# WISDEM/RAFT

Hardware: AMD Instinct MI355X
Metric: design-case-frequency solves/sec (whole node) (higher is better)
Workload: dtype f64

## Files before the change

raft_amd/_abi.py:

```python
import ctypes as C
import os

import numpy as np

NFIELD = 32
FLAG_CONVERGED = 1
FLAG_NAN = 2

_c_double_p = C.POINTER(C.c_double)
_c_i64_p = C.POINTER(C.c_int64)
_c_i32_p = C.POINTER(C.c_int32)
_vp = C.c_void_p

EXPORTS = (
    "raftx_version", "raftx_is_device", "raftx_ctx_create", "raftx_ctx_destroy",
    "raftx_last_error", "raftx_upload_designs", "raftx_upload_cases",
    "raftx_excitation", "raftx_linearize", "raftx_solve_dynamics",
    "raftx_solve_system", "raftx_last_kernel_ms",
    "raftx_solve_dynamics_device", "raftx_fetch_results", "raftx_debug_math", "raftx_debug_math_table", "raftx_last_solve_kernel", "raftx_device_synchronize", "raftx_motion_stats", "raftx_solve_system_resident", "raftx_qtf_slender", "raftx_channel_stats", "raftx_qtf_force", "raftx_set_linearisation_point", "raftx_fetch_linearisation_point",
    "raftx_build_designs", "raftx_fetch_strips", "raftx_fetch_statics", "raftx_channel_stats_poly", "raftx_qtf_slender_rows", "raftx_bem_excitation", "raftx_qtf_kay", "raftx_host_alloc", "raftx_host_free", "raftx_device_locality", "raftx_solve_dense",
    "raftx_sweep_stats",
    "raftx_sweep_submit",
    "raftx_sweep_prepare",
    "raftx_sweep_launch",
# ... 115 lines not shown
            L.raftx_modal_batch.argtypes = [_vp, C.c_int, _vp, _vp, _vp, _vp, _vp]
            L.raftx_modal_batch.restype = C.c_int
            L.raftx_modal_resident.argtypes = [_vp, _vp, _vp, _vp, _vp, _vp, _vp]
            L.raftx_modal_resident.restype = C.c_int
            L.raftx_sweep_modal.argtypes = [_vp, C.c_int, _vp, _vp, _vp, _vp, _vp, _vp]
            L.raftx_sweep_modal.restype = C.c_int
        self.has_mooring = all(hasattr(L, s) for s in MOORING_EXPORTS)
        if self.has_mooring:
            L.raftx_mooring_lines.argtypes = [_vp, C.c_int, C.c_int, _vp, _vp, C.c_double, _vp, _vp, _vp, _vp, _vp, _vp]
            L.raftx_mooring_lines.restype = C.c_int
            L.raftx_mooring_program.argtypes = [_vp, C.c_int, _vp, C.c_int, _vp, _vp]
            L.raftx_mooring_program.restype = C.c_int
            L.raftx_mooring_expand.argtypes = [_vp, C.c_int, _vp, _vp]
            L.raftx_mooring_expand.restype = C.c_int
            L.raftx_sweep_mooring.argtypes = [_vp, C.c_int, C.c_int, _vp, C.c_int, _vp, _vp, _vp, _vp, _vp]
            L.raftx_sweep_mooring.restype = C.c_int
        self.has_statics = all(hasattr(L, s) for s in STATICS_EXPORTS)
        if self.has_statics:
            L.raftx_mean_pose.argtypes = [_vp, C.c_int, C.c_int, _vp, _vp, C.c_double, _vp, _vp, _vp, _vp, _vp, C.c_int,
                                          _vp, _vp, _vp, _vp, _vp, _vp, _vp, _vp]
            L.raftx_mean_pose.restype = C.c_int
            L.raftx_sweep_mean_pose.argtypes = [_vp, C.c_int, C.c_int, _vp, C.c_int, _vp, _vp, _vp, _vp, C.c_int, _vp, _vp, _vp, _vp]
            L.raftx_sweep_mean_pose.restype = C.c_int
        self.has_current = all(hasattr(L, s) for s in CURRENT_EXPORTS)
        if self.has_current:
            L.raftx_current_loads.argtypes = [_vp, C.c_int, _vp, _vp, _vp, C.c_double, C.c_double, _vp]
            L.raftx_current_loads.restype = C.c_int
            L.raftx_sweep_current.argtypes = [_vp, C.c_int, C.c_int, _vp, _vp, _vp, C.c_double, _vp]
            L.raftx_sweep_current.restype = C.c_int
        self.has_qtfgen = all(hasattr(L, s) for s in QTFGEN_EXPORTS)
        if self.has_qtfgen:
            L.raftx_qtf_tables_build.argtypes = [_vp, C.c_int, _vp, _vp, _vp, _vp, _vp, _vp, _vp]
            L.raftx_qtf_tables_build.restype = C.c_int
            L.raftx_qtf_tables_build_variants.argtypes = [_vp, C.c_int, _vp, _vp, _vp, _vp]
            L.raftx_qtf_tables_build_variants.restype = C.c_int
            L.raftx_qtf_tables_counts.argtypes = [_vp, _vp]
            L.raftx_qtf_tables_counts.restype = C.c_int
            L.raftx_qtf_tables_fetch.argtypes = [_vp, _vp, _vp, _vp, _vp]
            L.raftx_qtf_tables_fetch.restype = C.c_int
            L.raftx_qtf_tables_kay_items.argtypes = [_vp, C.c_int, _vp, _vp, _vp]
            L.raftx_qtf_tables_kay_items.restype = C.c_int
            L.raftx_qtf_slender_resident.argtypes = [_vp, C.c_int, C.c_int, _vp, _vp, C.c_double, C.c_double, C.c_double, _vp, _vp,
                                                     _vp, C.c_int, _vp]
            L.raftx_qtf_slender_resident.restype = C.c_int
        self.has_channels = all(hasattr(L, s) for s in CHANNEL_EXPORTS)
        if self.has_channels:
# ... 345 lines not shown
                                                        float(XiStart), int(n_chunk), _ptr(out["std"]), _ptr(out["niter"]),
                                                        _ptr(out["flags"]), _ptr(out["Xi"]), _ptr(out["strip_off"]))
        self._check(rc, "raftx_sweep_prepare_variants")
        return dict(slot=int(slot), inputs=inputs, out=out)

    def sweep_launch(self, handle):
        self._check(self.rlib.lib.raftx_sweep_launch(self._h, int(handle["slot"])), "raftx_sweep_launch")
        return handle

    def sweep_submit(self, slot, *args, **kw):
        return self.sweep_launch(self.sweep_prepare(slot, *args, **kw))

    def sweep_wait(self, handle):
        out = handle["out"]
        self._check(self.rlib.lib.raftx_sweep_wait(self._h, int(handle["slot"]), _ptr(out["timing_ms"])), "raftx_sweep_wait")
        span = np.zeros(2)
        self._check(self.rlib.lib.raftx_sweep_solve_span(self._h, int(handle["slot"]), _ptr(span[0:1]), _ptr(span[1:2])),
                    "raftx_sweep_solve_span")
        out["solve_span_ms"] = span
        nf, nb = C.c_int(0), C.c_int(0)
        self._check(self.rlib.lib.raftx_sweep_generation(self._h, int(handle["slot"]), C.byref(nf), C.byref(nb)),
                    "raftx_sweep_generation")
        out["generation_fused_blocks"] = (nf.value, nb.value)
        handle["inputs"] = None
        return out

    def sweep_cancel(self, handle):
        self._check(self.rlib.lib.raftx_sweep_cancel(self._h, int(handle["slot"])), "raftx_sweep_cancel")
        handle["inputs"] = None

    def sweep_stats(self, tables, M0, B0, C0, w, k, depth, zeta, beta, nIter, tol=0.01, XiStart=0.1, pose=None,
                    rho=1025.0, g=9.81, rho_wave=1025.0, g_wave=9.81, add_mask=7, Fz_moor=None, n_chunk=0, n_worker=0,
                    want_Xi=False, Xi_out=None):
        self.resident_generation += 1
        nD, nC, nH, nw, inputs, out = self._sweep_prepare(tables, M0, B0, C0, w, k, depth, zeta, beta, pose, Fz_moor, want_Xi, Xi_out)
        (member_off, members, station_off, stations, cap_off, caps, pose, M0, B0, C0, Fz, w, k, zeta, beta) = inputs
        rc = self.rlib.lib.raftx_sweep_stats(self._h, nD, _ptr(member_off), _ptr(members), _ptr(station_off), _ptr(stations),
                                             _ptr(cap_off), _ptr(caps), _ptr(pose), float(rho), float(g), int(add_mask),
                                             _ptr(M0), _ptr(B0), _ptr(C0), _ptr(Fz), nC, nH, nw, _ptr(w), _ptr(k), float(depth),
                                             float(rho_wave), float(g_wave), _ptr(zeta), _ptr(beta), int(nIter), float(tol),
                                             float(XiStart), int(n_chunk), int(n_worker), _ptr(out["std"]), _ptr(out["niter"]),
                                             _ptr(out["flags"]), _ptr(out["Xi"]), _ptr(out["strip_off"]), _ptr(out["timing_ms"]))
        self._check(rc, "raftx_sweep_stats")
        return out

    def fetch_strips(self, n_strips, n_cm_rows=0):
# ... 819 lines not shown
```

raft_amd/csrc/build.py:

```python
import os
import subprocess
import sys

HERE = os.path.dirname(os.path.abspath(__file__))
SRC = os.path.join(HERE, "raftx_hip.hip")
OUT = os.path.join(HERE, "libraftx_hip.so")
FLAGS = ["--offload-arch=gfx950", "-O3", "-std=c++17", "-shared", "-fPIC", "-fno-gpu-rdc", "-mllvm", "-disable-machine-licm"]


def build(force=False, verbose=False, extra=()):
    deps = [SRC, os.path.join(HERE, "..", "..", "include", "raftx.h"), os.path.join(HERE, "..", "..", "include", "raftx_modal.h"),
            os.path.join(HERE, "..", "..", "include", "raftx_current.h"),
            os.path.join(HERE, "..", "..", "include", "raftx_channels.h"),
            os.path.join(HERE, "..", "..", "include", "raftx_qtfgen.h"),
            os.path.join(HERE, "..", "..", "include", "raftx_mooring.h"),
            os.path.join(HERE, "..", "..", "include", "raftx_statics.h"), os.path.abspath(__file__)]
    deps += [os.path.join(HERE, f) for f in os.listdir(HERE) if f.endswith(".h")]
    if (not force) and os.path.exists(OUT) and all(os.path.getmtime(OUT) >= os.path.getmtime(d) for d in deps):
        return OUT
    hipcc = os.environ.get("HIPCC", "hipcc")
    cmd = [hipcc] + FLAGS + list(extra) + ["-o", OUT, SRC]
    if verbose:
        print(" ".join(cmd))
    subprocess.check_call(cmd)
    return OUT


def build_timing(verbose=False):
    out = os.path.join(HERE, "libraftx_hip_timing.so")
    cmd = [os.environ.get("HIPCC", "hipcc")] + FLAGS + ["-DRAFTX_PHASE_TIMING", "-DGEOM_PHASE_TIMING", "-o", out, SRC]
    if verbose:
        print(" ".join(cmd))
    subprocess.check_call(cmd)
    return out


if __name__ == "__main__":
    if "--timing" in sys.argv:
        print(build_timing(verbose=True))
# ... 4 lines not shown
```

raft_amd/csrc/raftx_hip.hip:

```cpp

#include <hip/hip_runtime.h>
#include <rccl/rccl.h>
#include <dlfcn.h>

#include <algorithm>
#include <cmath>
#include <cstdint>
#include <cstdio>
#include <cstdlib>
#include <cstring>
#include <chrono>
#include <map>
#include <functional>
#include <limits>
#include <mutex>
#include <type_traits>
#include <thread>
#include <unordered_map>
#include <vector>

#include "../../include/raftx.h"
#include "../../include/raftx_modal.h"
#include "../../include/raftx_current.h"
#include "../../include/raftx_channels.h"
#include "../../include/raftx_qtfgen.h"
#include "../../include/raftx_mooring.h"
#include "../../include/raftx_statics.h"

struct Roctx {
    int (*push)(const char *) = nullptr;
    int (*pop)() = nullptr;
    Roctx() {
        if (getenv("RAFTX_NO_ROCTX")) return;
        for (const char *n : {"librocprofiler-sdk-roctx.so.1", "librocprofiler-sdk-roctx.so", "libroctx64.so.4", "libroctx64.so"}) {
            if (void *h = dlopen(n, RTLD_NOW | RTLD_LOCAL)) {
                push = reinterpret_cast<int (*)(const char *)>(dlsym(h, "roctxRangePushA"));
                pop = reinterpret_cast<int (*)()>(dlsym(h, "roctxRangePop"));
                if (push && pop) return;
                push = nullptr;
                pop = nullptr;
            }
        }
    }
};
static Roctx &roctx() {
    static Roctx r;
    return r;
}
struct RangeScope {
    bool on;
// ... 296 lines not shown
    const size_t t = (size_t)blockIdx.x * blockDim.x + threadIdx.x;
    if (t >= (size_t)npair * 36 * nw) return;
    const int iw = (int)(t % nw), e = (int)((t / nw) % 36);
    const size_t pair = t / ((size_t)36 * nw), d = pair / nCase;
    const double ww = w[iw], Bq = uB[d * 36 + e] + uBd[pair * 36 + e];
    Z[t] = {fma(-(ww * ww), uM[d * 36 + e], uC[d * 36 + e]), ww * Bq};
}

static int solve_system_shape(int n, int nRhs, size_t *lds) {
    const size_t per = sizeof(cplx) * (size_t)n * (n + nRhs);
    const int nbin = per * 4 <= 64 * 1024 ? 4 : (per * 2 <= 64 * 1024 ? 2 : 1);
    *lds = per * nbin;
    return nbin;
}

__global__ void __launch_bounds__(256) k_motion_stats(int npair, int nHead, int nw, double inv_dw,
                                                      const cplx *__restrict__ Xi, double *__restrict__ sd,
                                                      double *__restrict__ psd,
                                                      const int *__restrict__ niter = nullptr, const int *__restrict__ flags = nullptr,
                                                      int *__restrict__ ints_out = nullptr) {
    __shared__ double part[4][6];
    const int p = blockIdx.x;
    if (p >= npair) return;
    const double r2d = 180.0 / 3.14159265358979323846;
    double acc[6] = {0, 0, 0, 0, 0, 0};
    for (int i = threadIdx.x; i < nw; i += blockDim.x) {
#pragma unroll
        for (int j = 0; j < 6; j++) {
            const double scale = j >= 3 ? r2d : 1.0;
            double a2 = 0.0;
            for (int ih = 0; ih < nHead; ih++) {
                const cplx x = Xi[(((size_t)p * nHead + ih) * 6 + j) * nw + i];
                const double xr = x.re * scale, xi = x.im * scale;
                a2 += xr * xr + xi * xi;
            }
            acc[j] += a2;
            if (psd) psd[((size_t)p * 6 + j) * nw + i] = 0.5 * a2 * inv_dw;
        }
    }
    const int lane = threadIdx.x & 63, wv = threadIdx.x >> 6;
#pragma unroll
    for (int j = 0; j < 6; j++) {
        double a = acc[j];
        for (int o = 32; o > 0; o >>= 1) a += __shfl_xor(a, o, 64);
        if (lane == 0) part[wv][j] = a;
    }
    __syncthreads();
    if (threadIdx.x < 6) {
        double a = 0.0;
        for (int q = 0; q < (int)(blockDim.x >> 6); q++) a += part[q][threadIdx.x];
        sd[(size_t)p * 6 + threadIdx.x] = sqrt(0.5 * a);
    }
    if (ints_out && threadIdx.x == 6) {
        ints_out[p] = niter[p];
        ints_out[npair + p] = flags[p];
    }
}

// ... 242 lines not shown
};
struct VariantSrc {
    const VariantProg *prog;
    const double *params;
    const FixedRecord *rec = nullptr;
};

static void variant_view(const VariantProg &P, VariantView &V) {
    V.nM = P.nM; V.nSt = P.nSt; V.nCap = P.nCap; V.nP = P.nP;
    V.gm = P.gm; V.gs = P.gs; V.gc = P.gc;
    V.stMember = P.stMember; V.capMember = P.capMember;
    V.stFrac = P.stFrac; V.fillFrac = P.fillFrac; V.capFrac = P.capFrac;
    V.endCoef = P.endCoef; V.headCS = P.headCS; V.diaCoef = P.diaCoef;
    V.endEdit = P.endEdit; V.diaEdit = P.diaEdit;
}
static void expand_args(const VariantProg &P, int n, double *gm_out, double *gs_out, double *gc_out, ExpandArgs &E) {
    variant_view(P, E);
    E.n = n;
    E.gm_out = gm_out; E.gs_out = gs_out; E.gc_out = gc_out;
}
static bool fused_gen_asked() {
    const char *fg = getenv("RAFTX_FUSED_GEN");
    return fg && atoi(fg);
}

struct DenseResident {
    int nSet = 0, n = 0, nw = 0, freq_mask = 0;
    double *w = nullptr, *M = nullptr, *B = nullptr, *C = nullptr;
    Bag allocs;
};
struct QtfResident {
    bool valid = false;
    int nDesign = 0;
    std::vector<int64_t> off;
    int64_t *dOff = nullptr;
    double *strips = nullptr, *members = nullptr, *kay = nullptr;
    Bag allocs;
    int64_t total(int j) const { return off[(size_t)j * (nDesign + 1) + nDesign]; }
};
struct raftx_ctx;
struct DevOffsets {
    const int64_t *memberOff, *stationOff, *capOff;
};
struct SeaStates { int nCase, nHead, nw; const double *w, *k; double depth, rho, g; const double *zeta, *beta; };
struct BuildSource {
    const int64_t *memberOff, *stationOff, *capOff;
// ... 163 lines not shown
    DevTables T{};
    cplx *rXi = nullptr, *rFw = nullptr, *rZ = nullptr, *rFe = nullptr;
    double *rB = nullptr;
    int *rNi = nullptr, *rFl = nullptr;
    size_t r_npair = 0, r_nx = 0, r_nz = 0;
    int r_mask = 0;
    int r_last_mask = 0;
    bool r_fe = false;
    unsigned kpNext = 0;
    int nCU = 0;
    int last_flags = -1, last_minb = 0, last_rc = 0;
    int rQtf_sets = 0, rQtf_nw2 = 0, rKay_sets = 0, rKay_nw2 = 0;
    bool have_xl0 = false, want_xlout = false;
    int maxS = 0;
    std::vector<int> hS;
    double last_ms = 0.0;
    bool have_designs = false, have_cases = false;
    int nw_designs = 0;
    bool kay_ready = false, bem_ready = false;
    int g_n = 0;
    size_t g_nStrips = 0, g_nRows = 0;
    double *g_abi = nullptr, *g_A = nullptr, *g_Ch = nullptr, *g_Wh = nullptr, *g_props = nullptr, *g_Ms = nullptr, *g_Cs = nullptr, *g_Ws = nullptr;
    bool last_gen_fused = false;
    cplx *g_cm = nullptr;
    void *comm = nullptr;
    int comm_rank = 0, comm_world = 1;
    std::vector<raftx_ctx *> workers[RAFTX_NSLOT];
};

#define MAX_NW 2048
#define HIPCHK(ctx, call)                                                                              \
    do {                                                                                               \
        hipError_t e_ = (call);                                                                        \
        if (e_ != hipSuccess) {                                                                        \
            snprintf((ctx)->err, sizeof((ctx)->err), "%s failed: %s (%s:%d)", #call, hipGetErrorString(e_), \
                     __FILE__, __LINE__);                                                              \
            return -2;                                                                                 \
        }                                                                                              \
    } while (0)
#define FAIL(ctx, ...)                                        \
    do {                                                      \
        snprintf((ctx)->err, sizeof((ctx)->err), __VA_ARGS__); \
        return -1;                                            \
    } while (0)

extern "C" int raftx_version(void) { return RAFTX_VERSION; }
// ... 1072 lines not shown

static int fill_solve_args(raftx_ctx *c, int nIter, double tol, double XiStart, const raftx_c128 *F_extra, int want_mask, SolveArgs *out) {
    if (check_ready(c)) return -1;
    if (nIter < 0) FAIL(c, "solve_dynamics: nIter < 0");
    HIPCHK(c, hipSetDevice(c->device));
    if (ensure_results(c, want_mask, F_extra != nullptr)) return -1;
    SolveArgs &A = *out;
    A.nIter = nIter + 1;
    A.tol = tol;
    A.XiStart = XiStart;
    A.F_extra = F_extra ? c->rFe : (c->bem_ready ? c->bemF.p : nullptr);
    A.Xi = c->rXi;
    A.niter = c->rNi;
    A.flags = c->rFl;
    A.B_drag = (want_mask & RAFTX_WANT_BDRAG) ? c->rB : nullptr;
    A.F_wave = (want_mask & RAFTX_WANT_FWAVE) ? c->rFw : nullptr;
    A.Z = (want_mask & RAFTX_WANT_Z) ? c->rZ : nullptr;
    c->r_last_mask = want_mask;
    A.pairs = nullptr;
    A.npairs = 0;
    A.Xl0 = nullptr;
    A.XlOut = nullptr;
    A.dbg = nullptr;
#ifdef RAFTX_PHASE_TIMING
    const size_t ndbg = 10 + 2 * PT_CLOCK_BUCKETS;
    HIPCHK(c, c->dbg.zeroed_once(ndbg, c->stream));
    HIPCHK(c, hipMemsetAsync(c->dbg.p, 0, ndbg * sizeof(unsigned long long), c->stream));
    HIPCHK(c, hipMemsetAsync(c->dbg.p + 8, 0xFF, sizeof(unsigned long long), c->stream));
    A.dbg = c->dbg.p;
#endif
    if (F_extra && c->r_nx) H2D(c, c->rFe, F_extra, c->r_nx * sizeof(cplx));
    return 0;
}

static int solve_enqueue(raftx_ctx *c, int nIter, double tol, double XiStart, const raftx_c128 *F_extra, int want_mask,
                         SlabPlan *plan = nullptr) {
    SolveArgs A;
    if (int rc = fill_solve_args(c, nIter, tol, XiStart, F_extra, want_mask, &A)) return rc;
    LaunchPlan lp;
    if (int rc = make_plan(c, &A, &lp)) return rc;
    const size_t lds = lp.lds(c->maxS, A.rc_n);
    if (int rc = ensure_xl_scratch(c, lp)) return rc;
    A.Xl = c->rXl.p;
    A.slots = c->rXlSlots.p;
    if (c->have_xl0 || c->want_xlout) {
        const size_t nxl = c->r_npair * 6 * (size_t)c->T.nw;
        if (c->have_xl0 && c->rXl0.n != nxl) FAIL(c, "solve_dynamics: the linearisation point was set for a different batch shape");
        if (int rc = ensure_xlio(c, nxl)) return rc;
        if (c->have_xl0) A.Xl0 = c->rXl0.p;
        A.XlOut = c->rXlOut.p;
        c->have_xl0 = false;
    }
    LdsClasses classes;
    if (int rc = lds_classes(c, lp, &classes)) return rc;
    const bool slabbed = plan && classes.cls.empty() && !plan->alts.empty() && plan->bnd.size() >= 2 && plan->bnd.back() == c->r_npair;
    if (int rc = slabbed ? ensure_slab_list(c) : 0) return rc;
    const bool whole = classes.cls.empty() && !slabbed;
    const bool gen_fused = c->last_gen_fused = resolve_generation(c, lp, whole);
    if (prep_lds(c, reinterpret_cast<const void *>(lp.k.fn), lds)) return -1;
    HIPCHK(c, hipEventRecord(c->ev0, c->stream));
    int rc_after = 0;
    if (whole && launch_whole(c, lp, A, lds, gen_fused)) return -1;
    if (slabbed && launch_slabs(c, lp, A, lds, plan, &rc_after)) return -2;
    if (!classes.cls.empty()) launch_classes(c, lp, A, classes);
    if (plan && plan->after && !slabbed) rc_after = plan->after(0, c->r_npair, c->stream);
    HIPCHK(c, hipEventRecord(c->ev1, c->stream));
    HIPCHK(c, hipGetLastError());
    if (rc_after) FAIL(c, "solve_dynamics: what follows a slab of the launch could not be enqueued");
    return 0;
}
static int finish_enqueued(raftx_ctx *c) {
    HIPCHK(c, hipStreamSynchronize(c->stream));
    float ms = 0.f;
    HIPCHK(c, hipEventElapsedTime(&ms, c->ev0, c->ev1));
    c->last_ms = ms;
    return 0;
}
extern "C" int raftx_solve_dynamics_device(raftx_ctx *c, int nIter, double tol, double XiStart,
                                           const raftx_c128 *F_extra, int want_mask) {
    RangeScope range_("raftx_solve_dynamics_device: fused fixed point");
    const int rc = solve_enqueue(c, nIter, tol, XiStart, F_extra, want_mask);
// ... 756 lines not shown
static void cut_blocks(raftx_ctx *c, int slot, int nDesign, const SeaStates &sea, const SweepRun &run) {
    SweepSlot &S = c->slots[slot];
    S.bnd = sweep_bounds(nDesign, (long)nDesign * sea.nCase, std::min(run.nChunk, 64), others_in_flight(c, slot));
    S.dw = sea.nw > 1 ? sea.w[1] - sea.w[0] : sea.w[0];
    S.nIter = run.nIter; S.tol = run.tol; S.XiStart = run.XiStart;
    S.blk.assign(S.bnd.size() - 1, nullptr);
    S.nCase = sea.nCase; S.nHead = sea.nHead; S.nw = sea.nw;
    S.sd = run.sd; S.niter = run.niter; S.flags = run.flags; S.Xi = run.Xi; S.stripOffsets = run.stripOffsets;
    S.tl[0] = S.since();
    S.allocs.release();
    S.clear_requests();
}
static int upload_offsets(raftx_ctx *c, SweepSlot &S, const BuildSource &src, int nDesign) {
    S.p1 = src;
    S.p1.k_dev = c->csets[S.cset].T.k;
    const int64_t nMemberAll = src.memberOff[nDesign];
    DevOffsets &dOff = S.p1.dOff;
    int rc = upload_on(c, c->sCopy, S.allocs, src.memberOff, (size_t)nDesign + 1, &dOff.memberOff);
    rc |= upload_on(c, c->sCopy, S.allocs, src.stationOff, (size_t)nMemberAll + 1, &dOff.stationOff);
    if (src.capOff) rc |= upload_on(c, c->sCopy, S.allocs, src.capOff, (size_t)nMemberAll + 1, &dOff.capOff);
    return rc ? -2 : 0;
}
static int block_phase1(raftx_ctx *c, SweepSlot &S, size_t b) {
    return build_phase1(S.blk[b], c->sCopy, c->sPrep, S.p1, S.bnd[b], S.bnd[b + 1] - S.bnd[b]);
}

static void launch_mean_pose(hipStream_t st, MeanPoseArgs &A, int nDesign, int nLine, double depth, double tolT, double tolR, int max_iter);
static int block_pose(raftx_ctx *c, SweepSlot &S, size_t b) {
    raftx_ctx *sub = S.blk[b];
    BuildJob &J = sub->job;
    GeomArgs &A = J.A;
    const size_t lo = (size_t)S.bnd[b], nAll = (size_t)S.bnd.back();
    const int n = S.bnd[b + 1] - S.bnd[b];
    HIPCHK(sub, sub->evPose.ensure(hipEventDisableTiming));
    hipStream_t sPrep = c->sPrep;
    if (n > 0) {
        if (!J.active || J.nDesign != n) FAIL(sub, "sweep_mean_pose: the block has no member pass in flight (internal error)");
        HIPCHK(sub, hipStreamWaitEvent(sPrep, S.pose.evUp, 0));
        if (J.reduce_stream) HIPCHK(sub, hipStreamWaitEvent(sPrep, sub->evRed, 0));
        const auto &P = S.pose;
        PoseAssembleArgs Q;
        memset(&Q, 0, sizeof(Q));
        Q.n = n; Q.Cs = A.Cs; Q.Ch = A.Ch; Q.Ws = A.Ws; Q.Wh = A.Wh;
        Q.strideC = P.nX > 1 ? 36 : 0; Q.strideF = P.nX > 1 ? 6 : 0;
        Q.Cx = P.Cx ? P.Cx + lo * Q.strideC : nullptr;
        Q.Fx = P.Fx ? P.Fx + lo * Q.strideF : nullptr;
// ... 574 lines not shown
static int mooring_add_block(raftx_ctx *c, raftx_ctx *sub, SweepSlot &S, int lo, int n, bool pipelined) {
    if (!n) return 0;
    if (!sub->job.active || !sub->job.C0d) FAIL(sub, "sweep_mooring: the block has no uploaded C0 (internal error)");
    HIPCHK(sub, sub->evMoor.ensure(hipEventDisableTiming));
    hipLaunchKernelGGL(k_moor_add, dim3(moor_grid((long long)n * 36)), dim3(MOOR_THREADS), 0, c->sCopy, sub->job.C0d,
                       S.mooring.C + (size_t)lo * 36, (long long)n * 36);
    HIPCHK(sub, hipGetLastError());
    HIPCHK(sub, hipEventRecord(sub->evMoor, c->sCopy));
    HIPCHK(sub, hipStreamWaitEvent(c->stream, sub->evMoor, 0));
    if (pipelined && c->sGen) HIPCHK(sub, hipStreamWaitEvent(c->sGen, sub->evMoor, 0));
    return 0;
}

static hipStream_t download_stream(raftx_ctx *c) {
    (void)c->sD2Hhigh.ensure_highest(hipStreamNonBlocking);
    return c->sD2Hhigh ? c->sD2Hhigh : c->sD2H;
}

static int enqueue_stats(raftx_ctx *c, SweepSlot &S, size_t b, hipStream_t sDown) {
    raftx_ctx *sub = S.blk[b];
    const int lo = S.bnd[b], nCase = S.nCase, nHead = S.nHead, nw = S.nw;
    const size_t npair = (size_t)(S.bnd[b + 1] - lo) * nCase;
    hipError_t e = hipEventRecord(sub->evS0, c->stream);
    if (npair) {
        const landing::Stats land = landing::stats(npair);
        hipLaunchKernelGGL(k_motion_stats, dim3((unsigned)npair), bin_threads(nw), 0, c->stream,
                           (int)npair, nHead, nw, 1.0 / S.dw, sub->rXi, sub->pinRes.p + land.sd, (double *)nullptr, (const int *)sub->rNi,
                           (const int *)sub->rFl, land.niter.in(sub->pinRes.p));
    }
    if (e == hipSuccess) e = hipEventRecord(sub->evS1, c->stream);
    if (e == hipSuccess && S.modal.on) e = modal_block(sub, S, lo, S.bnd[b + 1] - lo, c->stream);
    if (e == hipSuccess && S.current.on) e = current_block(sub, S, lo, S.bnd[b + 1] - lo, c->csets[S.cset].T.depth, c->stream);
    if (e == hipSuccess && S.channels.on) e = channels_block(sub, S, lo, S.bnd[b + 1] - lo, c->stream);
    if (e == hipSuccess && S.mooring.on && S.mooring.Tstd_out) e = mooring_std_block(sub, S, lo, S.bnd[b + 1] - lo, c->stream);
    if (e == hipSuccess) e = hipEventRecord(sub->evDone, c->stream);
    if (e == hipSuccess && S.Xi && !S.slab) {
        e = hipStreamWaitEvent(sDown, sub->evDone, 0);
        if (e == hipSuccess && sub->r_nx)
            e = hipMemcpyAsync(S.Xi + (size_t)lo * nCase * nHead * 6 * nw, sub->rXi, sub->r_nx * sizeof(cplx), hipMemcpyDeviceToHost, sDown);
    }
    if (e != hipSuccess) {
        snprintf(sub->err, sizeof(sub->err), "statistics / download of the block: %s", hipGetErrorString(e));
        return -2;
    }
    return 0;
}

// ... 43 lines not shown
        if (sl != slot && c->slots[sl].prepared && !c->slots[sl].blk.empty() && c->slots[sl].blk[0])
            if (hipStreamWaitEvent(c->sGen, c->slots[sl].blk[0]->evZ, 0) != hipSuccess) return -2;
    return 0;
}
static void hand_sea_states(const DevTables &P, raftx_ctx *sub) {
    DevTables &T = sub->T;
    T.nCase = P.nCase; T.nHead = P.nHead; T.nw = P.nw;
    T.w = P.w; T.k = P.k; T.csh = P.csh; T.cch = P.cch; T.zeta = P.zeta; T.beta = P.beta;
    T.depth = P.depth; T.rho = P.rho; T.g = P.g;
    sub->have_cases = true;
}
static int launch_block(raftx_ctx *c, SweepSlot &S, int slot, size_t b, LaunchMode &M) {
    raftx_ctx *sub = S.blk[b];
    int rc = (S.mooring.on && S.mooring.add) ? mooring_add_block(c, sub, S, S.bnd[b], S.bnd[b + 1] - S.bnd[b], M.pipelined) : 0;
    if (!rc) rc = phase1_ahead(c, S, b);
    if (!rc && b == 0 && M.pipelined) rc = gate_generation(c, slot);
    S.tlb.push_back(S.since());
    const int kind = GEN_CROSSING | ((S.nCase == 1 && !S.slab && !S.current.on && !S.pose.on) ? GEN_MAY_DEFER : 0) | (M.pipelined ? GEN_PIPELINED : 0);
    if (!rc) rc = build_phase2(sub, nullptr, M.pipelined ? c->sGen : nullptr, kind);
    S.tlb.push_back(S.since());
    if (!rc) {
        hand_sea_states(c->csets[S.cset].T, sub);
        if (S.slab) slab_plan_block(M.plan, S, b, M.slab_pairs, M.sDown);
        rc = solve_enqueue(sub, S.nIter, S.tol, S.XiStart, nullptr, 0, S.slab ? &M.plan : nullptr);
    }
    if (!rc && sub->pinRes.reserve(landing::stats((size_t)(S.bnd[b + 1] - S.bnd[b]) * S.nCase).need) != hipSuccess) rc = -2;
    if (!rc && !S.slab) rc = enqueue_stats(c, S, b, M.sDown);
    S.tlb.push_back(S.since());
    if (rc) snprintf(c->err, sizeof(c->err), "sweep_stats (block %zu): %s", b, sub->err);
    return rc;
}
static int stats_after_join(raftx_ctx *c, SweepSlot &S, LaunchMode &M) {
    const size_t nB = S.blk.size();
    if (!nB) return 0;
    if (S.blk[0]->evJoin.ensure(hipEventDisableTiming) != hipSuccess) return -2;
    if (int rc = slab_join(S.blk[0], c->stream, M.plan.alts)) return rc;
    if (hipEventRecord(S.blk[nB - 1]->ev1, c->stream) != hipSuccess) return -2;
    for (size_t b = 0; b < nB; b++)
        if (int rc = enqueue_stats(c, S, b, M.sDown)) {
            snprintf(c->err, sizeof(c->err), "sweep_stats (block %zu): %s", b, S.blk[b]->err);
            return rc;
        }
    return 0;
}

extern "C" int raftx_sweep_launch(raftx_ctx *c, int slot) {
    RangeScope range_("raftx_sweep_launch: generation + fused fixed point + statistics (enqueue)");
    if (!c) return -1;
    SLOT_REF(S, c, slot, "sweep_launch");
// ... 157 lines not shown
    if (es != hipSuccess) S.clear_requests();
    HIPCHK(c, es);
    solve_span(c, S);
    double t[4] = {0, 0, 0, 0};
    if (S.stripOffsets) S.stripOffsets[0] = 0;
    for (size_t b = 0; b < S.blk.size(); b++) collect_block(S, b, t);
    const hipError_t em = collect_mooring(S);
    if (em == hipSuccess) collect_pose(S);
    S.clear_requests();
    HIPCHK(c, em);
    t[0] = S.since();
    debug_timeline(S, slot, t[0]);
    if (timing_ms) memcpy(timing_ms, t, sizeof(t));
    c->last_ms = t[2];
    return 0;
}

extern "C" int raftx_sweep_solve_span(raftx_ctx *c, int slot, double *start_ms, double *end_ms) {
    if (!c) return -1;
    SLOT_REF(S, c, slot, "sweep_solve_span");
    if (S.busy) FAIL(c, "sweep_solve_span: slot %d has not been waited for", slot);
    if (start_ms) *start_ms = S.span[0];
    if (end_ms) *end_ms = S.span[1];
    return 0;
}

extern "C" int raftx_sweep_generation(raftx_ctx *c, int slot, int *blocks_fused, int *blocks) {
    if (!c) return -1;
    SLOT_REF(S, c, slot, "sweep_generation");
    int nf = 0, nb = 0;
    for (raftx_ctx *sub : S.blk)
        if (sub) {
            nb++;
            nf += sub->last_gen_fused ? 1 : 0;
        }
    if (blocks_fused) *blocks_fused = nf;
    if (blocks) *blocks = nb;
    return 0;
}

static int modal_launch(raftx_ctx *c, int n, const double *M, const double *C, const double *dM, const double *dC,
                        const double *props_in, double *fn, double *modes, int32_t *flags, double *props) {
    Scratch sc(c);
    double *dfn = sc.out<double>(fn, (size_t)n * 6), *dmo = sc.out<double>(modes, (size_t)n * 36);
    int32_t *dfl = sc.out<int32_t>(flags, (size_t)n);
    double *dpr = sc.out<double>(props, (size_t)n * RAFTX_SP_N);
// ... 799 lines not shown
```

raft_amd/csrc/raftx_kernels.h:

```cpp
#pragma once
#include <type_traits>
#include "raftx_tables.h"

#define NF RAFTX_NFIELD

struct cplx {
    double re, im;
};
__device__ __forceinline__ cplx cmul(cplx a, cplx b) { return {a.re * b.re - a.im * b.im, a.re * b.im + a.im * b.re}; }
__device__ __forceinline__ cplx cscale(cplx a, double s) { return {a.re * s, a.im * s}; }
__device__ __forceinline__ cplx cadd(cplx a, cplx b) { return {a.re + b.re, a.im + b.im}; }
__device__ __forceinline__ cplx csub(cplx a, cplx b) { return {a.re - b.re, a.im - b.im}; }

#define CONST_AS __attribute__((address_space(4)))
typedef const CONST_AS double *cdptr;
typedef const CONST_AS int *ciptr;
#define LDS_AS __attribute__((address_space(3)))
typedef LDS_AS double *ldptr;
typedef LDS_AS int *liptr;
__device__ __forceinline__ cdptr as_const(const double *p) { return (cdptr)p; }
__device__ __forceinline__ ciptr as_const(const int *p) { return (ciptr)p; }

#pragma clang fp contract(off)
__device__ __forceinline__ void fast_sincos(double x, double &s, double &c) {
// ... 2299 lines not shown
        for (int a = 0; a < 3; a++)
            Fexc[((size_t)s * 3 + a) * nw + iw] = {Bm[a * 3] * u[0].re + Bm[a * 3 + 1] * u[1].re + Bm[a * 3 + 2] * u[2].re,
                                                   Bm[a * 3] * u[0].im + Bm[a * 3 + 1] * u[1].im + Bm[a * 3 + 2] * u[2].im};
    }
}

struct SolveArgs {
    int nIter;
    double tol, XiStart;
    const cplx *__restrict__ F_extra;
    cplx *Xi;
    int *__restrict__ niter, *__restrict__ flags;
    double *__restrict__ B_drag;
    cplx *__restrict__ F_wave;
    cplx *__restrict__ Z;
    double *Xl;
    unsigned long long *slots;
    const cplx *__restrict__ Xl0;
    cplx *__restrict__ XlOut;
    unsigned long long *dbg;
    const int *__restrict__ pairs;
    int npairs;
    int rc_n;
};

#define KP_STASH 4
template <int NB, int FLAGS, int MAXT, bool PERSIST>
__device__ __forceinline__ void solve_pair(const DevTables &T, const SolveArgs &A, int idx, unsigned xslot) {
    extern __shared__ __attribute__((aligned(16))) double smem[];
    constexpr bool FDEP = (FLAGS & KF_FDEP) != 0, OUTZ = (FLAGS & KF_OUTZ) != 0, OUTF = (FLAGS & KF_OUTF) != 0;
    constexpr bool EXTRA = (FLAGS & KF_EXTRA) != 0, MCF = (FLAGS & KF_MCF) != 0, MULTI = (FLAGS & KF_MULTI) != 0;
    constexpr bool XLIO = (FLAGS & KF_XLIO) != 0;
    PairCtx p;
    {
        const int nl = A.pairs ? A.npairs : T.nDesign * T.nCase;
        if (idx >= nl) return;
        if (!pair_ctx(T, p, A.pairs ? A.pairs[idx] : idx)) return;
    }
    PT_DECL;
    PT_BEGIN(A);
    const bool multi = blockDim.x > 64;
    const int nw = T.nw, nHs = T.nHead, nH = MULTI ? T.nHead : 1;
    const int pair = p.pair, S = p.S;
    const cplx *cm = (MCF && T.cm) ? p.cm : nullptr;
    constexpr int STAGE = stage_policy(NB, MAXT);
    constexpr bool XLG = xl_global(NB, MAXT);
    constexpr int PARK = park_policy(NB, MAXT);
    constexpr bool RC = PARK != 0 && (XLG || RAFTX_XL_LDS);
    Lds l = carve(smem + (PERSIST ? KP_STASH : 0), S, XLG ? 0 : nw, blockDim.x >> 6, STAGE, PARK, RC ? A.rc_n : 0, RC ? nw : 0);
// ... 289 lines not shown
#pragma unroll
            for (int j = 0; j < NB; j++) {
                const int ib = j * blockDim.x + opaque((int)threadIdx.x);
                const bool act = ib < nw;
                const int iw = act ? ib : 0;
                const double wl = T.w[iw];
                cplx y[6];
#pragma unroll
                for (int q = 0; q < 6; q++) y[q] = j == 0 ? x[0][q] : xo[(size_t)q * nw + iw];
                assemble_and_solve<(FLAGS & ~KF_OUTZ)>(l, mb, nw, iw, act ? wl : 0.0, y, nullptr, act);
                if (act) {
#pragma unroll
                    for (int q = 0; q < 6; q++) xo[(size_t)q * nw + iw] = nan ? cplx{NAN, NAN} : y[q];
                }
            }
        }
    }
    PT_MARK(5);
    PT_FLUSH(A);
    if (threadIdx.x < 36 && A.B_drag) A.B_drag[(size_t)pair * 36 + threadIdx.x] = l.Bd[threadIdx.x];
    if (threadIdx.x == 0) {
        if (A.niter) A.niter[pair] = done;
        if (A.flags) A.flags[pair] = (converged ? RAFTX_FLAG_CONVERGED : 0) | (nan ? RAFTX_FLAG_NAN : 0);
    }
}

template <int NB, int FLAGS, int MAXT, int MINB>
__global__ void __launch_bounds__(MAXT, MINB) k_solve_dynamics(DevTables T, SolveArgs A) {
    const int nl = A.pairs ? A.npairs : T.nDesign * T.nCase;
    solve_pair<NB, FLAGS, MAXT, false>(T, A, pair_of_block(blockIdx.x, nl), 0u);
}

#define KP_CTR_STRIDE 32
struct PersistArgs {
    DevTables T;
    SolveArgs A;
    unsigned *ctr;
    unsigned xl_base;
};
__device__ __forceinline__ void kp_leave(const PersistArgs &P) {
    if (threadIdx.x == 0) {
        unsigned *left = P.ctr + 8 * KP_CTR_STRIDE;
        const unsigned n = __hip_atomic_fetch_add(left, 1u, __ATOMIC_RELAXED, __HIP_MEMORY_SCOPE_AGENT);
        if (n + 1 == gridDim.x) {
            for (int x = 0; x < 9; x++) __hip_atomic_store(P.ctr + x * KP_CTR_STRIDE, 0u, __ATOMIC_RELAXED, __HIP_MEMORY_SCOPE_AGENT);
        }
    }
}
__device__ __forceinline__ int claim_pair(unsigned *ctr, int nl, LDS_AS int *mail) {
    __syncthreads();
    if (threadIdx.x == 0) {
        unsigned xcc;
        asm volatile("s_getreg_b32 %0, hwreg(HW_REG_XCC_ID)" : "=s"(xcc));
        xcc &= 7u;
        const int per = (nl + 7) >> 3;
        int idx = -1;
        for (unsigned t = 0; t < 8u && idx < 0; t++) {
            const unsigned x = (xcc + t) & 7u;
            const int lim = min(per, nl - (int)x * per);
            if (lim <= 0) continue;
            unsigned *cx = ctr + x * KP_CTR_STRIDE;
            if ((int)__hip_atomic_load(cx, __ATOMIC_RELAXED, __HIP_MEMORY_SCOPE_AGENT) >= lim) continue;
// ... 31 lines not shown
                     : "v"(threadIdx.x), "v"((unsigned)(size_t)(LDS_AS double *)smem)                                   \
                     : "memory", "v0", "v1", "v2", "v3", "v4", "v5", "v6", "v7", "s0", "s1", "s2", "s3", "s4", "s5",    \
                       "s6", "s8", "s9");                                                                               \
        __builtin_unreachable();                                                                                        \
    } while (0)
#define RAFTX_KP_DEFINE(NAME, NB, FLAGS, MAXT, MINB)                                                                    \
    extern "C" __global__ void __launch_bounds__(MAXT, MINB) NAME(PersistArgs P) {                                      \
        extern __shared__ __attribute__((aligned(16))) double smem[];                                                   \
        if (threadIdx.x == 0) {                                                                                         \
            LDS_AS unsigned *st_ = (LDS_AS unsigned *)smem;                                                             \
            const size_t qp_ = (size_t)__builtin_amdgcn_queue_ptr(), ka_ = (size_t)__builtin_amdgcn_kernarg_segment_ptr(); \
            st_[1] = blockIdx.x + 0u * (blockIdx.y + blockIdx.z + threadIdx.y + threadIdx.z);                           \
            st_[2] = (unsigned)qp_;                                                                                     \
            st_[3] = (unsigned)(qp_ >> 32);                                                                             \
            st_[4] = (unsigned)ka_;                                                                                     \
            st_[5] = (unsigned)(ka_ >> 32);                                                                             \
        }                                                                                                               \
        const int nl = P.A.pairs ? P.A.npairs : P.T.nDesign * P.T.nCase;                                                \
        const int idx = claim_pair(P.ctr, nl, (LDS_AS int *)smem);                                                      \
        if (idx < 0) {                                                                                                  \
            kp_leave(P);                                                                                                \
            return;                                                                                                     \
        }                                                                                                               \
        solve_pair<NB, FLAGS, MAXT, true>(P.T, P.A, idx, P.xl_base + blockIdx.x);                                       \
        RAFTX_KP_REENTER(NAME);                                                                                         \
    }
#ifndef RAFTX_KP_MINB
#define RAFTX_KP_MINB 2
#endif
#define X(F) RAFTX_KP_DEFINE(raftx_kp_f##F, 2, F, 128, RAFTX_KP_MINB)
#ifdef RAFTX_KP_ONLY
X(0)
#else
RAFTX_PERSIST128(X)
#endif
#undef X
```

Before: 707.1 million.

## Fuse motion statistics into persistent solve kernel epilogue

Adds an epilogue to the persistent solver kernel that computes per-pair motion standard deviations and writes iteration counts and flags straight into the pinned landing buffer. When fusion applies (single heading, whole-run persistent launch, non-multi kernel), the separate k_motion_stats launch is skipped. The aim is to drop a kernel launch and a second read of Xi from global memory. In exchange it adds extra work, LDS use and syncs to every persistent block, and the epilogue assumes 2 waves of 128 threads and at most 256 frequency bins.

```diff
diff --git a/include/raftx_stats_form.h b/include/raftx_stats_form.h
--- /dev/null
+++ b/include/raftx_stats_form.h
@@ -0,0 +1,15 @@
+#ifndef RAFTX_STATS_FORM_H
+#define RAFTX_STATS_FORM_H
+
+#include "raftx.h"
+
+#ifdef __cplusplus
+extern "C" {
+#endif
+
+int raftx_sweep_stats_form(raftx_ctx *ctx, int slot, int *blocks_fused, int *blocks);
+
+#ifdef __cplusplus
+}
+#endif
+#endif
diff --git a/raft_amd/_abi.py b/raft_amd/_abi.py
--- a/raft_amd/_abi.py
+++ b/raft_amd/_abi.py
@@ -161,6 +161,10 @@
             L.raftx_mean_pose.restype = C.c_int
             L.raftx_sweep_mean_pose.argtypes = [_vp, C.c_int, C.c_int, _vp, C.c_int, _vp, _vp, _vp, _vp, C.c_int, _vp, _vp, _vp, _vp]
             L.raftx_sweep_mean_pose.restype = C.c_int
+        self.has_stats_form = hasattr(L, "raftx_sweep_stats_form")
+        if self.has_stats_form:
+            L.raftx_sweep_stats_form.argtypes = [_vp, C.c_int, _vp, _vp]
+            L.raftx_sweep_stats_form.restype = C.c_int
         self.has_current = all(hasattr(L, s) for s in CURRENT_EXPORTS)
         if self.has_current:
             L.raftx_current_loads.argtypes = [_vp, C.c_int, _vp, _vp, _vp, C.c_double, C.c_double, _vp]
@@ -552,6 +556,10 @@
         self._check(self.rlib.lib.raftx_sweep_generation(self._h, int(handle["slot"]), C.byref(nf), C.byref(nb)),
                     "raftx_sweep_generation")
         out["generation_fused_blocks"] = (nf.value, nb.value)
+        if self.rlib.has_stats_form:
+            self._check(self.rlib.lib.raftx_sweep_stats_form(self._h, int(handle["slot"]), C.byref(nf), C.byref(nb)),
+                        "raftx_sweep_stats_form")
+            out["stats_fused_blocks"] = (nf.value, nb.value)
         handle["inputs"] = None
         return out
 
diff --git a/raft_amd/csrc/build.py b/raft_amd/csrc/build.py
--- a/raft_amd/csrc/build.py
+++ b/raft_amd/csrc/build.py
@@ -14,7 +14,8 @@
             os.path.join(HERE, "..", "..", "include", "raftx_channels.h"),
             os.path.join(HERE, "..", "..", "include", "raftx_qtfgen.h"),
             os.path.join(HERE, "..", "..", "include", "raftx_mooring.h"),
-            os.path.join(HERE, "..", "..", "include", "raftx_statics.h"), os.path.abspath(__file__)]
+            os.path.join(HERE, "..", "..", "include", "raftx_statics.h"),
+            os.path.join(HERE, "..", "..", "include", "raftx_stats_form.h"), os.path.abspath(__file__)]
     deps += [os.path.join(HERE, f) for f in os.listdir(HERE) if f.endswith(".h")]
     if (not force) and os.path.exists(OUT) and all(os.path.getmtime(OUT) >= os.path.getmtime(d) for d in deps):
         return OUT
diff --git a/raft_amd/csrc/raftx_hip.hip b/raft_amd/csrc/raftx_hip.hip
--- a/raft_amd/csrc/raftx_hip.hip
+++ b/raft_amd/csrc/raftx_hip.hip
@@ -26,6 +26,7 @@
 #include "../../include/raftx_qtfgen.h"
 #include "../../include/raftx_mooring.h"
 #include "../../include/raftx_statics.h"
+#include "../../include/raftx_stats_form.h"
 
 struct Roctx {
     int (*push)(const char *) = nullptr;
@@ -368,18 +369,12 @@
     __shared__ double part[4][6];
     const int p = blockIdx.x;
     if (p >= npair) return;
-    const double r2d = 180.0 / 3.14159265358979323846;
     double acc[6] = {0, 0, 0, 0, 0, 0};
     for (int i = threadIdx.x; i < nw; i += blockDim.x) {
 #pragma unroll
         for (int j = 0; j < 6; j++) {
-            const double scale = j >= 3 ? r2d : 1.0;
             double a2 = 0.0;
-            for (int ih = 0; ih < nHead; ih++) {
-                const cplx x = Xi[(((size_t)p * nHead + ih) * 6 + j) * nw + i];
-                const double xr = x.re * scale, xi = x.im * scale;
-                a2 += xr * xr + xi * xi;
-            }
+            for (int ih = 0; ih < nHead; ih++) a2 += motion_stats_term(Xi[(((size_t)p * nHead + ih) * 6 + j) * nw + i], j);
             acc[j] += a2;
             if (psd) psd[((size_t)p * 6 + j) * nw + i] = 0.5 * a2 * inv_dw;
         }
@@ -668,6 +663,10 @@
 static bool fused_gen_asked() {
     const char *fg = getenv("RAFTX_FUSED_GEN");
     return fg && atoi(fg);
+}
+static bool fused_stats_asked() {
+    const char *fs = getenv("RAFTX_FUSED_STATS");
+    return fs ? atoi(fs) != 0 : true;
 }
 
 struct DenseResident {
@@ -877,6 +876,7 @@
     size_t g_nStrips = 0, g_nRows = 0;
     double *g_abi = nullptr, *g_A = nullptr, *g_Ch = nullptr, *g_Wh = nullptr, *g_props = nullptr, *g_Ms = nullptr, *g_Cs = nullptr, *g_Ws = nullptr;
     bool last_gen_fused = false;
+    bool last_stats_fused = false;
     cplx *g_cm = nullptr;
     void *comm = nullptr;
     int comm_rank = 0, comm_world = 1;
@@ -1995,6 +1995,8 @@
     A.Xl0 = nullptr;
     A.XlOut = nullptr;
     A.dbg = nullptr;
+    A.sd = nullptr;
+    A.ints_out = nullptr;
 #ifdef RAFTX_PHASE_TIMING
     const size_t ndbg = 10 + 2 * PT_CLOCK_BUCKETS;
     HIPCHK(c, c->dbg.zeroed_once(ndbg, c->stream));
@@ -2006,8 +2008,9 @@
     return 0;
 }
 
+struct StatsLanding { double *sd; int *ints; };
 static int solve_enqueue(raftx_ctx *c, int nIter, double tol, double XiStart, const raftx_c128 *F_extra, int want_mask,
-                         SlabPlan *plan = nullptr) {
+                         SlabPlan *plan = nullptr, const StatsLanding *landing = nullptr) {
     SolveArgs A;
     if (int rc = fill_solve_args(c, nIter, tol, XiStart, F_extra, want_mask, &A)) return rc;
     LaunchPlan lp;
@@ -2030,6 +2033,12 @@
     if (int rc = slabbed ? ensure_slab_list(c) : 0) return rc;
     const bool whole = classes.cls.empty() && !slabbed;
     const bool gen_fused = c->last_gen_fused = resolve_generation(c, lp, whole);
+    c->last_stats_fused = landing && whole && lp.k.kp && !gen_fused && lp.lean >= 0 && !(lp.lean & KF_MULTI) && c->T.nHead == 1 &&
+                          fused_stats_asked();
+    if (c->last_stats_fused) {
+        A.sd = landing->sd;
+        A.ints_out = landing->ints;
+    }
     if (prep_lds(c, reinterpret_cast<const void *>(lp.k.fn), lds)) return -1;
     HIPCHK(c, hipEventRecord(c->ev0, c->stream));
     int rc_after = 0;
@@ -2832,6 +2841,10 @@
     return rc ? -2 : 0;
 }
 static int block_phase1(raftx_ctx *c, SweepSlot &S, size_t b) {
+    if (S.blk[b]->pinRes.reserve(landing::stats((size_t)(S.bnd[b + 1] - S.bnd[b]) * S.nCase).need) != hipSuccess) {
+        snprintf(S.blk[b]->err, sizeof(S.blk[b]->err), "sweep_prepare: no page-locked memory for the block's statistics");
+        return -2;
+    }
     return build_phase1(S.blk[b], c->sCopy, c->sPrep, S.p1, S.bnd[b], S.bnd[b + 1] - S.bnd[b]);
 }
 
@@ -3452,7 +3465,7 @@
     const int lo = S.bnd[b], nCase = S.nCase, nHead = S.nHead, nw = S.nw;
     const size_t npair = (size_t)(S.bnd[b + 1] - lo) * nCase;
     hipError_t e = hipEventRecord(sub->evS0, c->stream);
-    if (npair) {
+    if (npair && !sub->last_stats_fused) {
         const landing::Stats land = landing::stats(npair);
         hipLaunchKernelGGL(k_motion_stats, dim3((unsigned)npair), bin_threads(nw), 0, c->stream,
                            (int)npair, nHead, nw, 1.0 / S.dw, sub->rXi, sub->pinRes.p + land.sd, (double *)nullptr, (const int *)sub->rNi,
@@ -3542,9 +3555,13 @@
     if (!rc) {
         hand_sea_states(c->csets[S.cset].T, sub);
         if (S.slab) slab_plan_block(M.plan, S, b, M.slab_pairs, M.sDown);
-        rc = solve_enqueue(sub, S.nIter, S.tol, S.XiStart, nullptr, 0, S.slab ? &M.plan : nullptr);
-    }
-    if (!rc && sub->pinRes.reserve(landing::stats((size_t)(S.bnd[b + 1] - S.bnd[b]) * S.nCase).need) != hipSuccess) rc = -2;
+    }
+    const landing::Stats land = landing::stats((size_t)(S.bnd[b + 1] - S.bnd[b]) * S.nCase);
+    if (!rc && sub->pinRes.reserve(land.need) != hipSuccess) rc = -2;
+    if (!rc) {
+        const StatsLanding out{sub->pinRes.p + land.sd, land.niter.in(sub->pinRes.p)};
+        rc = solve_enqueue(sub, S.nIter, S.tol, S.XiStart, nullptr, 0, S.slab ? &M.plan : nullptr, &out);
+    }
     if (!rc && !S.slab) rc = enqueue_stats(c, S, b, M.sDown);
     S.tlb.push_back(S.since());
     if (rc) snprintf(c->err, sizeof(c->err), "sweep_stats (block %zu): %s", b, sub->err);
@@ -3748,6 +3765,20 @@
     if (S.busy) FAIL(c, "sweep_solve_span: slot %d has not been waited for", slot);
     if (start_ms) *start_ms = S.span[0];
     if (end_ms) *end_ms = S.span[1];
+    return 0;
+}
+
+extern "C" int raftx_sweep_stats_form(raftx_ctx *c, int slot, int *blocks_fused, int *blocks) {
+    if (!c) return -1;
+    SLOT_REF(S, c, slot, "sweep_stats_form");
+    int nf = 0, nb = 0;
+    for (raftx_ctx *sub : S.blk)
+        if (sub) {
+            nb++;
+            nf += sub->last_stats_fused ? 1 : 0;
+        }
+    if (blocks_fused) *blocks_fused = nf;
+    if (blocks) *blocks = nb;
     return 0;
 }
 
diff --git a/raft_amd/csrc/raftx_kernels.h b/raft_amd/csrc/raftx_kernels.h
--- a/raft_amd/csrc/raftx_kernels.h
+++ b/raft_amd/csrc/raftx_kernels.h
@@ -2345,9 +2345,29 @@
     const int *__restrict__ pairs;
     int npairs;
     int rc_n;
+    double *sd;
+    int *ints_out;
 };
 
 #define KP_STASH 4
+#define KP_CTR_STRIDE 32
+struct PersistArgs {
+    DevTables T;
+    SolveArgs A;
+    unsigned *ctr;
+    unsigned xl_base;
+};
+__device__ __forceinline__ const CONST_AS PersistArgs *kp_stashed_args(const double *smem) {
+    LDS_AS unsigned *st = (LDS_AS unsigned *)smem;
+    const unsigned lo = __builtin_amdgcn_readfirstlane(st[4]), hi = __builtin_amdgcn_readfirstlane(st[5]);
+    return (const CONST_AS PersistArgs *)(((size_t)hi << 32) | lo);
+}
+
+__device__ __forceinline__ double motion_stats_term(cplx x, int dof) {
+    const double r2d = 180.0 / 3.14159265358979323846;
+    const double xr = dof >= 3 ? __dmul_rn(x.re, r2d) : x.re, xi = dof >= 3 ? __dmul_rn(x.im, r2d) : x.im;
+    return fma(xr, xr, __dmul_rn(xi, xi));
+}
 template <int NB, int FLAGS, int MAXT, bool PERSIST>
 __device__ __forceinline__ void solve_pair(const DevTables &T, const SolveArgs &A, int idx, unsigned xslot) {
     extern __shared__ __attribute__((aligned(16))) double smem[];
@@ -2683,6 +2703,61 @@
     if (threadIdx.x == 0) {
         if (A.niter) A.niter[pair] = done;
         if (A.flags) A.flags[pair] = (converged ? RAFTX_FLAG_CONVERGED : 0) | (nan ? RAFTX_FLAG_NAN : 0);
+        if constexpr (PERSIST && !MULTI) {
+            const CONST_AS PersistArgs *P = kp_stashed_args(smem);
+            if (int *out = P->A.ints_out) {
+                out[pair] = done;
+                out[P->T.nDesign * P->T.nCase + pair] = (converged ? RAFTX_FLAG_CONVERGED : 0) | (nan ? RAFTX_FLAG_NAN : 0);
+            }
+        }
+    }
+}
+
+__device__ __forceinline__ void kp_stats_epilogue(double *smem) {
+    const CONST_AS PersistArgs *P = kp_stashed_args(smem);
+    double *sd = P->A.sd;
+    if (!sd) return;
+    const int pair = __builtin_amdgcn_readfirstlane(((LDS_AS int *)smem)[6]);
+    const int nw = P->T.nw, tid = threadIdx.x, lane = tid & 63, wv = tid >> 6;
+    const cplx *xi = P->A.Xi + (size_t)pair * 6 * nw;
+    cplx x[2][6];
+#pragma unroll
+    for (int j = 0; j < 2; j++) {
+        const int i = j * 128 + tid;
+#pragma unroll
+        for (int q = 0; q < 6; q++) x[j][q] = cplx{0.0, 0.0};
+        if (i < nw) {
+#pragma unroll
+            for (int q = 0; q < 6; q++) x[j][q] = xi[(size_t)q * nw + i];
+        }
+    }
+    double acc[2][6];
+#pragma unroll
+    for (int j = 0; j < 2; j++)
+#pragma unroll
+        for (int q = 0; q < 6; q++) {
+            double a2 = 0.0;
+            a2 += motion_stats_term(x[j][q], q);
+            acc[j][q] = 0.0 + a2;
+        }
+#pragma unroll
+    for (int j = 0; j < 2; j++)
+#pragma unroll
+        for (int q = 0; q < 6; q++)
+            for (int o = 32; o > 0; o >>= 1) acc[j][q] += __shfl_xor(acc[j][q], o, 64);
+    ldptr part = (ldptr)(smem + KP_STASH);
+    __syncthreads();
+    if (lane == 0) {
+#pragma unroll
+        for (int j = 0; j < 2; j++)
+#pragma unroll
+            for (int q = 0; q < 6; q++) part[(2 * j + wv) * 6 + q] = acc[j][q];
+    }
+    __syncthreads();
+    if (tid < 6) {
+        double a = 0.0;
+        for (int v = 0; v < 4; v++) a += part[v * 6 + tid];
+        sd[(size_t)pair * 6 + tid] = sqrt(0.5 * a);
     }
 }
 
@@ -2692,13 +2767,6 @@
     solve_pair<NB, FLAGS, MAXT, false>(T, A, pair_of_block(blockIdx.x, nl), 0u);
 }
 
-#define KP_CTR_STRIDE 32
-struct PersistArgs {
-    DevTables T;
-    SolveArgs A;
-    unsigned *ctr;
-    unsigned xl_base;
-};
 __device__ __forceinline__ void kp_leave(const PersistArgs &P) {
     if (threadIdx.x == 0) {
         unsigned *left = P.ctr + 8 * KP_CTR_STRIDE;
@@ -2776,7 +2844,12 @@
             kp_leave(P);                                                                                                \
             return;                                                                                                     \
         }                                                                                                               \
+        if constexpr (!((FLAGS) & KF_MULTI)) {                   \
+            static_assert(NB == 2 && MAXT == 128, "kp_stats_epilogue is written for two waves of two bins a lane");    \
+            if (threadIdx.x == 0) ((LDS_AS int *)smem)[6] = idx;                                                        \
+        }                                                                                                               \
         solve_pair<NB, FLAGS, MAXT, true>(P.T, P.A, idx, P.xl_base + blockIdx.x);                                       \
+        if constexpr (!((FLAGS) & KF_MULTI)) kp_stats_epilogue(smem);                                                   \
         RAFTX_KP_REENTER(NAME);                                                                                         \
     }
 #ifndef RAFTX_KP_MINB
```

After: 713.8 million, median of 6. Within noise of the previous version (+0.9%).
